# HpWang-whu/YOHO

Hardware: AMD Instinct MI355X
Metric: keypoints/sec (5000 kp x60 rot desc+YOHO-O) (higher is better)
Workload: dtype fp16x2 split (2^-22-accurate products, fp32 accumulate); 1 GPU

## Files before the change

yoho_amd/csrc/api.hip:

```cpp
#include "common.h"
#include <cstdarg>
#include <cstdio>
#include <cstring>
#include <cstdlib>
#include <cmath>
#include <vector>

namespace yoho {

static thread_local char g_err[512] = "";

void set_error(const char* fmt, ...) {
    va_list ap;
    va_start(ap, fmt);
    vsnprintf(g_err, sizeof(g_err), fmt, ap);
    va_end(ap);
}

void clear_error() { g_err[0] = 0; }

int hip_fail(hipError_t e, const char* what, const char* file, int line) {
    set_error("HIP error %d (%s) at %s:%d: %s", (int)e, hipGetErrorString(e), file, line, what);
    return YOHO_EHIP;
}
// ... 280 lines not shown
                const int g = outg[cfg * G + sl];
                slab[cfg * NTAP * G + tap * nslots + sl] = (g < 0 ? 0 : (int)N[g * NTAP + tap]) * 1024;
            }
    };
    std::vector<int> all(G); for (int i = 0; i < G; ++i) all[i] = i;
    std::vector<int> one(NTAP); for (int k = 0; k < NTAP; ++k) one[k] = N[k];
    std::vector<bool> in2(G, false);
    for (int k = 0; k < NTAP; ++k) for (int k2 = 0; k2 < NTAP; ++k2) in2[N[one[k] * NTAP + k2]] = true;
    std::vector<int> two; for (int g = 0; g < G; ++g) if (in2[g]) two.push_back(g);
    if (two.size() > 48) { set_error("2-hop cone of group element 0 has %zu > 48 elements", two.size()); delete c; return YOHO_EINVAL; }
    fill(CFG_FULL, all, 15, false);
    fill(CFG_C45, two, 12, false);
    fill(CFG_C13, one, 4, false);
    fill(CFG_C1, std::vector<int>{0}, 1, true);
    if ((rc = upload_slot_tables(slab.data(), outg.data(), c->tabs)) || (rc = gconv_init())) { delete c; return rc; }
    {
        std::vector<int> slab4(3 * 7 * 32, 0), unitg(3 * 32 * 2, -1);
        const std::vector<int>* lists[3] = {&all, &two, &one};
        for (int cfg = 0; cfg < 3; ++cfg) {
            const std::vector<int>& gl = *lists[cfg];
            int* ug = &unitg[cfg * 64];
            for (size_t k = 0; k < gl.size(); ++k) ug[k] = gl[k];
            for (int tp = 0; tp < 7; ++tp)
                for (int u = 0; u < 32; ++u)
                    for (int gs = 0; gs < 2; ++gs)
                        for (int h = 0; h < 2; ++h) {
                            int g = ug[2 * u + gs];
                            if (g < 0) g = ug[2 * u];
                            int tap = 2 * tp + h;
                            if (tap >= NTAP) tap = 2 * tp;
                            slab4[(cfg * 7 + tp) * 32 + u] |= (g < 0 ? 0 : (int)N[g * NTAP + tap]) << (8 * (2 * gs + h));
                        }
        }
        if ((rc = upload_slot_tables16(slab4.data(), unitg.data(), c->tabs)) || (rc = gconv16_init())) { delete c; return rc; }
    }
    c->gconv_mode = 4;
    c->partII_mode = 2;
    {
        auto is = [](const char* name, const char* val) { const char* e = std::getenv(name); return e && std::strcmp(e, val) == 0; };
        auto num = [](const char* name) { const char* e = std::getenv(name); return e ? std::atoi(e) : 0; };
        c->env.partII_tail_staged = is("YOHO_PARTII_TAIL", "staged");
        c->env.transfer_staged = is("YOHO_TRANSFER", "staged");
        c->env.xf_steal = !is("YOHO_XF_STEAL", "0");
        c->env.nn_splits = num("YOHO_NN_SPLITS");
        c->env.spconv_debug = num("YOHO_SPCONV_DEBUG");
        c->env.fcgf_f32 = is("YOHO_FCGF", "f32");
        c->env.fcgf_full_maps = is("YOHO_FCGF_MAPS", "full");
        c->env.fcgf_norm_staged = is("YOHO_FCGF_NORM", "staged");
        c->env.fcgf_heads_staged = is("YOHO_FCGF_HEADS", "staged");
        if (const char* e = std::getenv("YOHO_WS_LIMIT_MB")) c->env.ws_limit_mb = std::atoll(e);
        if (is("YOHO_PARTII_L1", "3")) c->env.partII_l1_variant = FG_TILE256_W8;
    }
    if (const char* m = std::getenv("YOHO_FCGF_CELLS")) c->fcgf_cell_sort = std::atoi(m);
    if (const char* m = std::getenv("YOHO_FCGF_SORT")) c->fcgf_parity_sort = std::strcmp(m, "0") == 0 ? 0 : 1;
    if (const char* m = std::getenv("YOHO_FCGF_COORDS")) c->fcgf_hash_coords = std::strcmp(m, "hash") == 0 ? 1 : 0;
    if (const char* m = std::getenv("YOHO_NN")) c->nn_prefilter = std::strcmp(m, "brute") == 0 ? 0 : 1;
    if (const char* m = std::getenv("YOHO_PARTII")) c->partII_mode = std::strcmp(m, "f32") == 0 ? 0 : (std::strcmp(m, "fp16x2") == 0 ? 2 : (std::strcmp(m, "cgemm") == 0 ? 3 : (std::strcmp(m, "cgemm8") == 0 ? 4 : 1)));
    if (const char* m = std::getenv("YOHO_PARTI_CHUNK")) {
        int ck = 0, ns = 1;
        if (std::sscanf(m, "%dx%d", &ck, &ns) >= 1 && ck >= 0 && (ns == 1 || ns == 2)) { c->partI_chunk = (ck + 255) / 256 * 256; c->partI_streams = ns; }
    }
    if (const char* m = std::getenv("YOHO_GCONV")) c->gconv_mode = std::strcmp(m, "f32") == 0 ? 0 : (std::strcmp(m, "bf16x3") == 0 ? 1 : (std::strcmp(m, "fp16x2") == 0 ? 3 : (std::strcmp(m, "fgemm") == 0 ? 4 : (std::strcmp(m, "fgemm256") == 0 ? 5 : (std::strcmp(m, "fgemm128") == 0 ? 6 : (std::strcmp(m, "fgemm8") == 0 ? 7 : 2))))));
    c->fb = new FourierBasis();
    if ((rc = build_fourier(N, P, *c->fb))) { delete c->fb; delete c; return rc; }
    {
        std::vector<float> fpad(2 * 64 * 64, 0.f);
        for (int s = 0; s < G; ++s)
// ... 839 lines not shown
```

yoho_amd/csrc/common.h:

```cpp
#pragma once
#include <hip/hip_runtime.h>
#include <stdint.h>
#include <stddef.h>
#include <initializer_list>
#include "yoho_hip.h"
#include "arena.h"

namespace yoho {

constexpr int G = 60;
constexpr int NTAP = 13;
constexpr int F = 32;
constexpr int TILE = 32;
constexpr int SLAB_FLOATS = 2 * TILE * 4;
constexpr int CHUNK_FLOATS = G * SLAB_FLOATS;

void set_error(const char* fmt, ...);
void clear_error();
inline bool yoho_misaligned(std::initializer_list<const void*> ps, unsigned mask) {
    for (const void* p : ps) if ((reinterpret_cast<uintptr_t>(p) & mask) != 0) return true;
    return false;
}
#define YOHO_NEED_ALIGNED(fn, mask, ...)                                                                                  \
    do {                                                                                                                  \
// ... 91 lines not shown
int gft_init();
int fgemm_init();
size_t fgemm_planes_bytes(int kppad, int cin);
void fgemm_qinfo(int* qi);
void fgemm_plane_offsets(int kppad, int cin, long long* off);
int pack_fgemm_weights(const FourierBasis& fb, const float* W, int cin, int cout, std::vector<unsigned short>& out, float* descale,
                       std::vector<unsigned short>* out8 = nullptr);
int pack_cgemm_weights(const float* W, int cin, int cout, int ntaps, std::vector<unsigned short>& out, float* descale, std::vector<unsigned short>& out8);
int cgemm_init();
int launch_cgemm(const Layer& L, const char* Bstages, int nslot, const unsigned char* slot, const unsigned char* outg, int nT32, int nTiles16,
                 char* out, hipStream_t s, int* rflag, const unsigned* amax);
int launch_gft16_invg(const float* in, float* res0, char* planesG, const int* slot_of, int nslot, const void* Ffrag, const float* bn_s,
                      const float* bn_t, int nTiles, int C8, int nCU, hipStream_t s, int* rflag, unsigned* amax);
int launch_fgemm(const Layer& L, const char* Bplanes, int kppad, int nT32, const float* res, float* out, int flags, hipStream_t s,
                 int* rflag = nullptr, FGemmBlocking blocking = FG_TILE128, const unsigned* amax = nullptr);
void build_gft16_frags(const FourierBasis& fb, std::vector<unsigned short>& out);
int gconv_layer(yoho_ctx* c, const float* x, int B, int cin, int cout, const float* W, const float* bias, int transpose, float* y,
                hipStream_t s);
int bn_stats(const float* x, int B, int C, float* mean, float* var, hipStream_t s);
int bn_relu_apply(const float* x, int B, int C, const float* scale, const float* shift, float* y, hipStream_t s);
int bn_relu_backward(const float* x, const float* y, const float* dy, int B, int C, const float* gamma, const float* mean, const float* rstd,
                     int batch_stats, float* dx, float* dgamma, float* dbeta, hipStream_t s);
int gconv_wgrad(yoho_ctx* c, const float* x, const float* dy, int B, int cin, int cout, float* dW, float* db, hipStream_t s);
struct FcgfNet;
int fcgf_load(FcgfNet** out, const yoho_fcgf_config* cfg, const float* const* t, int ntensors, bool f32_kernels);
void fcgf_free(FcgfNet* n);
int fcgf_forward(yoho_ctx* ctx, const FcgfNet* net, const int* coords0, int n0, const int* off_host, int nb, float* out, hipStream_t s);
int fcgf_voxelize(yoho_ctx* ctx, const double* pts, int n, const double* R_host, double voxel, int64_t* sel, int* coords, float* pts_sel,
                  int* count_host, hipStream_t s);
int fcgf_rotate_select(const double* pts, const double* R_host, const int64_t* sel, int m, float* out, hipStream_t s);
int fcgf_voxelize_batch(yoho_ctx* ctx, const double* pts, int n, const double* R_host, int nb, double voxel, int64_t* sel, int* coords,
                        float* pts_sel, int* counts_host, hipStream_t s);
int launch_cone1(const Layer& L, const char* X, int nTiles32, int nTiles16, const float* res, float* out, const int* n0, hipStream_t s, float* part = nullptr);
int gft16_init();
int launch_gft16(const float* in, float* out32, char* planes, int kppad, const void* Ffrag, const float* bn_s, const float* bn_t, int nTiles,
                 int C8, int nCU, hipStream_t s, int B = 0, int* rflag = nullptr, int variant = 2, int* ctr = nullptr, unsigned* amax = nullptr);
int launch_gft16_invp(const float* in, float* res0, char* planes16, int nTiles16, const void* Ffrag, const float* bn_s, const float* bn_t,
                      int nTiles, int C8, int nCU, hipStream_t s, int* rflag = nullptr);
int launch_head2(const float* s0, const float* s1, const float* s2, const float* s3, const int64_t* pre_idx, const int* P, const float* bn_s,
                 const float* bn_t, int M, int nTiles, char* planes, int kppad, const void* Ffrag, hipStream_t s,
                 const int64_t* const* ridx = nullptr, int istride = 1, int* rflag = nullptr);
int launch_head16(const float* x, int B, int nTiles, char* planes, int kppad, const void* Ffrag, hipStream_t s, const float* x1 = nullptr,
                  int B0 = 0, int* rflag = nullptr);
int launch_gconvf(const Layer& L, const float* X, int nTiles, const float* res, float* out, int flags, hipStream_t s);
int launch_gft(int mode, const float* in, float* out, const float* Fpad, const float* bn_s, const float* bn_t, int nTiles, int C8, hipStream_t s);
int upload_slot_tables16(const int* slab4_h, const int* unitg_h, SlotTables& t);
int gconv16_init();
int launch_gconv16(const Layer& L, const char* X, int nTiles, const float* res, float* out_raw, char* out_act, int flags, hipStream_t s,
                   int cfg = 0, float* out_raw32 = nullptr, float* out_act32 = nullptr, int npl = 3, int* rflag = nullptr);
int launch_pack16_partII(const float* s0, const float* s1, const float* s2, const float* s3, const int64_t* pre_idx, const int* P,
                         const float* bn_s, const float* bn_t, int M, int nTiles16, char* out, hipStream_t s, int npl = 3, int* rflag = nullptr);
int launch_pack16_partI(const float* x, int B, int nTiles, char* out, hipStream_t s, int npl = 3, int* rflag = nullptr);
int launch_group_mean_np(const float* eqv, int B, float* out, hipStream_t s);
int launch_pack_partII(const float* s0, const float* s1, const float* s2, const float* s3, const int64_t* pre_idx,
                       const int* P, const float* bn_s, const float* bn_t, int M, int nTiles, float* out, hipStream_t s);
int launch_quat_norm(const float* y, int M, float* quat, hipStream_t s);

struct MfArgs {
    const float* a; const float* b;
    int Na, Nb;
    float* na2; float* nb2;
    _Float16* a16; _Float16* b16;
    unsigned* rowmin; unsigned* colmin;
    unsigned long long* keysA; unsigned long long* keysB;
    unsigned* maxn2;
    int* bad;
// ... 159 lines not shown
```

yoho_amd/csrc/cone1.hip:

```cpp
#include <hip/hip_runtime.h>
#include <type_traits>

#include "common.h"

namespace yoho {

typedef float floatx16 __attribute__((ext_vector_type(16)));
typedef float floatx4 __attribute__((ext_vector_type(4)));
typedef unsigned uintx4 __attribute__((ext_vector_type(4)));
typedef _Float16 halfx8 __attribute__((ext_vector_type(8)));
typedef const __attribute__((address_space(1))) void* gptr_t;
typedef __attribute__((address_space(3))) void* lptr_t;

constexpr int C1_CHUNK = 30720;
constexpr int C1_PLANE = 15360;
constexpr int C1_STAGE = 2 * 2 * 14 * 256;
constexpr int C1_UNITS = C1_STAGE / 1024;

struct Cone1Args {
    const char* X;
    const char* Wp;
    const float* bias;
    const float* res;
    float* out;
    int nTiles32, nTiles16, cin8, cout8;
    float* part;
    float descale;
    int n0[14];
};

__device__ __forceinline__ floatx16 mfma_c1(uintx4 a, uintx4 b, floatx16 c) {
    union { uintx4 u; halfx8 h; } ca, cb;
    ca.u = a; cb.u = b;
    return __builtin_amdgcn_mfma_f32_32x32x16_f16(ca.h, cb.h, c, 0, 0, 0);
}

template <int I, int N, typename Fn>
__device__ __forceinline__ void sfor_c1(Fn&& fn) {
    if constexpr (I < N) { fn(std::integral_constant<int, I>{}); sfor_c1<I + 1, N>(fn); }
}

__global__ __launch_bounds__(256, 1) void cone1_kernel(Cone1Args a) {
    __shared__ __attribute__((aligned(16))) char smem[3 * C1_STAGE];
    __shared__ int n0s[16];
    const int tid = threadIdx.x, lane = tid & 63;
    const int w = __builtin_amdgcn_readfirstlane(tid >> 6);
    const int nog = a.cout8 / 16;
    const int cn = a.cin8 / (int)gridDim.y, c0 = (int)blockIdx.y * cn;
    const int tile32 = blockIdx.x / nog, og = blockIdx.x - tile32 * nog;
    const int ob = og * 4 + w;
    if (tid < 14) n0s[tid] = a.n0[tid];
    __syncthreads();

    long long soff[4];
#pragma unroll
    for (int i = 0; i < 4; ++i) {
        const int u = w + 4 * i < C1_UNITS ? w + 4 * i : w + 4 * (i - 1);
        const int slot = u * 4 + (lane >> 4);
        const int pl = slot / 28, r = slot - pl * 28, ht = r / 14, k = r - ht * 14;
        int t16 = 2 * tile32 + ht;
        t16 = t16 < a.nTiles16 ? t16 : a.nTiles16 - 1;
        soff[i] = (long long)t16 * a.cin8 * C1_CHUNK + pl * C1_PLANE + n0s[k] * 256 + (lane & 15) * 16;
    }
    auto stage = [&](int c8, char* dst) {
#pragma unroll
        for (int i = 0; i < 4; ++i) {
            const int u = w + 4 * i < C1_UNITS ? w + 4 * i : w + 4 * (i - 1);
            __builtin_amdgcn_global_load_lds((gptr_t)(a.X + soff[i] + (long long)(c0 + c8) * C1_CHUNK), (lptr_t)(dst + u * 1024), 16, 0, 0);
        }
    };

    floatx16 acc[3];
#pragma unroll
    for (int j = 0; j < 3; ++j)
#pragma unroll
        for (int r = 0; r < 16; ++r) acc[j][r] = 0.f;

    const int lane_b = ((lane >> 4) & 1) * (14 * 256) + (lane >> 5) * 256 + (lane & 15) * 16;
    const uintx4* Wl = reinterpret_cast<const uintx4*>(a.Wp) + (size_t)ob * a.cin8 * (7 * 2 * 64) + lane;

    constexpr int RING = 3;
    uintx4 wreg[RING][7][2];
    auto loadW = [&](int c8, uintx4 (&wr)[7][2]) {
        const uintx4* Wn = Wl + (size_t)(c0 + c8) * (7 * 2 * 64);
#pragma unroll
        for (int tp = 0; tp < 7; ++tp) { wr[tp][0] = Wn[(tp * 2) * 64]; wr[tp][1] = Wn[(tp * 2 + 1) * 64]; }
    };
    auto compute = [&](const char* cur, const uintx4 (&wr)[7][2]) {
        const unsigned base = (unsigned)(size_t)(cur + lane_b);
        uintx4 bh[7], bl[7];
#pragma unroll
        for (int tp = 0; tp < 7; ++tp)
            asm volatile("ds_read_b128 %0, %2 offset:%3\n\tds_read_b128 %1, %2 offset:%4"
                         : "=&v"(bh[tp]), "=&v"(bl[tp]) : "v"(base), "n"(tp * 512), "n"(tp * 512 + 2 * 14 * 256) : "memory");
        asm volatile("s_waitcnt lgkmcnt(0)"
                     : "+v"(bh[0]), "+v"(bh[1]), "+v"(bh[2]), "+v"(bh[3]), "+v"(bh[4]), "+v"(bh[5]), "+v"(bh[6]),
                       "+v"(bl[0]), "+v"(bl[1]), "+v"(bl[2]), "+v"(bl[3]), "+v"(bl[4]), "+v"(bl[5]), "+v"(bl[6]) :: "memory");
#pragma unroll
        for (int tp = 0; tp < 7; ++tp) {
            acc[0] = mfma_c1(wr[tp][1], bh[tp], acc[0]);
            acc[1] = mfma_c1(wr[tp][0], bl[tp], acc[1]);
            acc[2] = mfma_c1(wr[tp][0], bh[tp], acc[2]);
        }
    };
    auto top = [&]() {
        __builtin_amdgcn_s_waitcnt(0x4F72);
        asm volatile("s_waitcnt lgkmcnt(0)" ::: "memory");
        __builtin_amdgcn_s_barrier();
        __builtin_amdgcn_sched_barrier(0);
    };
    auto stage_of = [&](int c8) { return smem + (c8 % RING) * C1_STAGE; };
    const int last = cn - 1;
    auto clamp = [&](int c8) { return c8 <= last ? c8 : last; };
    loadW(clamp(0), wreg[0]); stage(clamp(0), stage_of(0));
    loadW(clamp(1), wreg[1]); stage(clamp(1), stage_of(1));
    const int nmain = (cn / RING) * RING;
    for (int c8 = 0; c8 < nmain; c8 += RING) {
        sfor_c1<0, RING>([&](auto jc) {
            constexpr int jj = decltype(jc)::value;
            const int c = c8 + jj;
            top();
            loadW(clamp(c + RING - 1), wreg[(jj + RING - 1) % RING]);
            stage(clamp(c + RING - 1), stage_of(c + RING - 1));
            compute(stage_of(c), wreg[jj]);
        });
    }
    sfor_c1<0, RING - 1>([&](auto jc) {
        constexpr int jj = decltype(jc)::value;
        if (nmain + jj <= last) {
            top();
            loadW(last, wreg[(jj + RING - 1) % RING]);
            stage(last, stage_of(nmain + jj + RING - 1));
            compute(stage_of(nmain + jj), wreg[jj]);
        }
    });
    asm volatile("s_waitcnt vmcnt(0)" ::: "memory");

    const int kp32 = lane & 31, half = lane >> 5;
#pragma unroll
    for (int q = 0; q < 4; ++q) {
        const int ch = ob * 32 + q * 8 + half * 4;
        floatx4 val;
        val.x = (acc[0][4 * q + 0] + acc[1][4 * q + 0]) + acc[2][4 * q + 0];
        val.y = (acc[0][4 * q + 1] + acc[1][4 * q + 1]) + acc[2][4 * q + 1];
        val.z = (acc[0][4 * q + 2] + acc[1][4 * q + 2]) + acc[2][4 * q + 2];
        val.w = (acc[0][4 * q + 3] + acc[1][4 * q + 3]) + acc[2][4 * q + 3];
        if (gridDim.y > 1) {
            *reinterpret_cast<floatx4*>(a.part + ((((size_t)blockIdx.y * a.nTiles32 + tile32) * a.cout8 + ob * 4 + q) * 64 + lane) * 4) = val;
            continue;
        }
        val *= a.descale;
        val += *reinterpret_cast<const floatx4*>(a.bias + ch);
        const size_t off = (((((size_t)tile32 * a.cout8 + ob * 4 + q) * G + 0) * 2 + half) * TILE + kp32) * 4;
        if (a.res) val += *reinterpret_cast<const floatx4*>(a.res + off);
        *reinterpret_cast<floatx4*>(a.out + off) = val;
    }
}

int launch_cone1(const Layer& L, const char* X, int nTiles32, int nTiles16, const float* res, float* out, const int* n0, hipStream_t s, float* part) {
    if (L.cout_pad % 128 || !L.wph || L.cin % 32) { set_error("cone1: needs cout %% 128 == 0, cin %% 32 == 0 and fp16x2 weights"); return YOHO_EINVAL; }
    Cone1Args a;
    a.X = X; a.Wp = reinterpret_cast<const char*>(L.wph); a.bias = L.bias; a.res = res; a.out = out; a.part = part;
    if (part && (L.cin / 8) % 2) { set_error("cone1: K split needs an even number of channel chunks"); return YOHO_EINVAL; }
    a.nTiles32 = nTiles32; a.nTiles16 = nTiles16; a.cin8 = L.cin / 8; a.cout8 = L.cout_pad / 8; a.descale = L.wph_descale;
    for (int k = 0; k < 13; ++k) a.n0[k] = n0[k];
    a.n0[13] = n0[0];
    if (nTiles32 == 0) return 0;
    hipLaunchKernelGGL(cone1_kernel, dim3(nTiles32 * (a.cout8 / 16), part ? 2 : 1), dim3(256), 0, s, a);
    HIPCHK(hipGetLastError());
    return 0;
}

}
```

yoho_amd/csrc/gconv.hip:

```cpp
#include "common.h"

namespace yoho {

typedef float floatx16 __attribute__((ext_vector_type(16)));
typedef float floatx4 __attribute__((ext_vector_type(4)));

constexpr int CHUNK_BYTES = CHUNK_FLOATS * 4;
constexpr int LDS_BYTES = 2 * CHUNK_BYTES;

typedef const __attribute__((address_space(4))) int* cint_p;

int upload_slot_tables(const int* slab_h, const int* outg_h, SlotTables& t) {
    HIPCHK(hipMalloc((void**)&t.slabtab, sizeof(int) * NCFG * NTAP * G));
    HIPCHK(hipMalloc((void**)&t.outg, sizeof(int) * NCFG * G));
    HIPCHK(hipMemcpy(t.slabtab, slab_h, sizeof(int) * NCFG * NTAP * G, hipMemcpyHostToDevice));
    HIPCHK(hipMemcpy(t.outg, outg_h, sizeof(int) * NCFG * G, hipMemcpyHostToDevice));
    return 0;
}

typedef const __attribute__((address_space(1))) void* gptr_t;
typedef __attribute__((address_space(3))) void* lptr_t;

__device__ __forceinline__ void stage_chunk(const float* src, char* dst, int w, int lane, int npieces) {
    for (int p = w; p < npieces; p += 4) {
// ... 88 lines not shown
template <int GPW, bool OSPLIT>
static int launch_t(const ConvArgs& a, int flags, int nstage, int cfg, hipStream_t s) {
    const int grid = a.nTiles * a.nOB;
    hipLaunchKernelGGL((gconv_kernel<GPW, OSPLIT>), dim3(grid), dim3(256), LDS_BYTES, s, a, flags, nstage, cfg);
    HIPCHK(hipGetLastError());
    return 0;
}

template <int GPW, bool OSPLIT>
static int init_t() {
    HIPCHK(hipFuncSetAttribute(reinterpret_cast<const void*>(&gconv_kernel<GPW, OSPLIT>),
                               hipFuncAttributeMaxDynamicSharedMemorySize, LDS_BYTES));
    return 0;
}

struct MlpArgs {
    const float* X;
    const float *WA, *biasA, *sA, *tA;
    const float *WB, *biasB, *sB, *tB;
    const float *WC, *biasC;
    int cinA8, obA, obB, M;
    float* quat;
    const float* part; const float* biasP; const float* resP; float descaleP; int nTiles;
};

__device__ __forceinline__ floatx4 quat_unit(floatx4 q) {
#pragma clang fp contract(off)
    const float n = sqrtf(((q.x * q.x + q.y * q.y) + q.z * q.z) + q.w * q.w);
    floatx4 o;
    o.x = q.x / n; o.y = q.y / n; o.z = q.z / n; o.w = q.w / n;
    return o;
}

__global__ __launch_bounds__(256, 1) void mlp_head_kernel(MlpArgs a) {
    extern __shared__ __attribute__((aligned(16))) char smem[];
    const int tid = threadIdx.x, lane = tid & 63;
    const int w = __builtin_amdgcn_readfirstlane(tid >> 6);
    const int tile = blockIdx.x;
    char* sX = smem;
    char* sA = sX + a.cinA8 * 1024;
    char* sB = sA + a.obA * 4 * 1024;
    const int half = lane >> 5;
    if (a.part) {
        for (int p = w; p < a.cinA8; p += 4) {
            const size_t o0 = (((size_t)tile * a.cinA8 + p) * 64 + lane) * 4, o1 = o0 + (size_t)a.nTiles * a.cinA8 * 256;
            floatx4 val = *reinterpret_cast<const floatx4*>(a.part + o0) + *reinterpret_cast<const floatx4*>(a.part + o1);
            val *= a.descaleP;
            val += *reinterpret_cast<const floatx4*>(a.biasP + p * 8 + half * 4);
            if (a.resP) val += *reinterpret_cast<const floatx4*>(a.resP + ((size_t)tile * a.cinA8 + p) * CHUNK_FLOATS + lane * 4);
            *reinterpret_cast<floatx4*>(sX + p * 1024 + lane * 16) = val;
        }
    } else {
        const float* Xt = a.X + (size_t)tile * a.cinA8 * CHUNK_FLOATS;
        for (int p = w; p < a.cinA8; p += 4)
            __builtin_amdgcn_global_load_lds((gptr_t)(Xt + (size_t)p * CHUNK_FLOATS + lane * 4), (lptr_t)(sX + p * 1024), 16, 0, 0);
    }
    {
        floatx16 acc[4];
#pragma unroll
        for (int j = 0; j < 4; ++j)
#pragma unroll
            for (int i = 0; i < 16; ++i) acc[j][i] = 0.f;
        const floatx4* W0 = reinterpret_cast<const floatx4*>(a.WA) + (size_t)w * a.cinA8 * 64 + lane;
        const size_t wstride = (size_t)4 * a.cinA8 * 64;
        floatx4 wn[4];
#pragma unroll
        for (int j = 0; j < 4; ++j) wn[j] = W0[j * wstride];
        asm volatile("s_waitcnt vmcnt(0)" ::: "memory");
        __syncthreads();
        for (int c8 = 0; c8 < a.cinA8; ++c8) {
            floatx4 wc[4];
#pragma unroll
            for (int j = 0; j < 4; ++j) wc[j] = wn[j];
            if (c8 + 1 < a.cinA8) {
#pragma unroll
                for (int j = 0; j < 4; ++j) wn[j] = W0[j * wstride + (size_t)(c8 + 1) * 64];
            }
            const floatx4 xf = *reinterpret_cast<const floatx4*>(sX + c8 * 1024 + lane * 16);
#pragma unroll
            for (int j = 0; j < 4; ++j) {
                acc[j] = __builtin_amdgcn_mfma_f32_32x32x2f32(wc[j].x, xf.x, acc[j], 0, 0, 0);
                acc[j] = __builtin_amdgcn_mfma_f32_32x32x2f32(wc[j].y, xf.y, acc[j], 0, 0, 0);
                acc[j] = __builtin_amdgcn_mfma_f32_32x32x2f32(wc[j].z, xf.z, acc[j], 0, 0, 0);
                acc[j] = __builtin_amdgcn_mfma_f32_32x32x2f32(wc[j].w, xf.w, acc[j], 0, 0, 0);
            }
        }
#pragma unroll
        for (int j = 0; j < 4; ++j) {
            const int ob = w + 4 * j;
#pragma unroll
            for (int q = 0; q < 4; ++q) {
                const int ch = ob * 32 + q * 8 + half * 4;
                floatx4 val;
                val.x = acc[j][4 * q + 0]; val.y = acc[j][4 * q + 1];
                val.z = acc[j][4 * q + 2]; val.w = acc[j][4 * q + 3];
                val += *reinterpret_cast<const floatx4*>(a.biasA + ch);
                const floatx4 sc = *reinterpret_cast<const floatx4*>(a.sA + ch);
                const floatx4 sh = *reinterpret_cast<const floatx4*>(a.tA + ch);
                floatx4 y = val * sc + sh;
                y.x = fmaxf(y.x, 0.f); y.y = fmaxf(y.y, 0.f); y.z = fmaxf(y.z, 0.f); y.w = fmaxf(y.w, 0.f);
                *reinterpret_cast<floatx4*>(sA + (ob * 4 + q) * 1024 + lane * 16) = y;
            }
        }
    }
    __syncthreads();
    {
        floatx16 acc;
#pragma unroll
        for (int i = 0; i < 16; ++i) acc[i] = 0.f;
        const int cin8 = a.obA * 4;
        const floatx4* W0 = reinterpret_cast<const floatx4*>(a.WB) + (size_t)w * cin8 * 64 + lane;
        floatx4 wr[4];
#pragma unroll
        for (int d = 0; d < 4; ++d) wr[d] = W0[(size_t)(d < cin8 ? d : cin8 - 1) * 64];
        for (int c0 = 0; c0 < cin8; c0 += 4) {
#pragma unroll
            for (int d = 0; d < 4; ++d) {
                const int c8 = c0 + d;
                const floatx4 wc = wr[d];
                const int nx = c8 + 4 < cin8 ? c8 + 4 : cin8 - 1;
                wr[d] = W0[(size_t)nx * 64];
                const floatx4 xf = *reinterpret_cast<const floatx4*>(sA + c8 * 1024 + lane * 16);
                acc = __builtin_amdgcn_mfma_f32_32x32x2f32(wc.x, xf.x, acc, 0, 0, 0);
                acc = __builtin_amdgcn_mfma_f32_32x32x2f32(wc.y, xf.y, acc, 0, 0, 0);
                acc = __builtin_amdgcn_mfma_f32_32x32x2f32(wc.z, xf.z, acc, 0, 0, 0);
                acc = __builtin_amdgcn_mfma_f32_32x32x2f32(wc.w, xf.w, acc, 0, 0, 0);
            }
        }
#pragma unroll
        for (int q = 0; q < 4; ++q) {
            const int ch = w * 32 + q * 8 + half * 4;
            floatx4 val;
            val.x = acc[4 * q + 0]; val.y = acc[4 * q + 1];
            val.z = acc[4 * q + 2]; val.w = acc[4 * q + 3];
            val += *reinterpret_cast<const floatx4*>(a.biasB + ch);
            const floatx4 sc = *reinterpret_cast<const floatx4*>(a.sB + ch);
            const floatx4 sh = *reinterpret_cast<const floatx4*>(a.tB + ch);
            floatx4 y = val * sc + sh;
            y.x = fmaxf(y.x, 0.f); y.y = fmaxf(y.y, 0.f); y.z = fmaxf(y.z, 0.f); y.w = fmaxf(y.w, 0.f);
            *reinterpret_cast<floatx4*>(sB + (w * 4 + q) * 1024 + lane * 16) = y;
        }
    }
    __syncthreads();
    if (w == 0) {
        floatx16 acc;
#pragma unroll
        for (int i = 0; i < 16; ++i) acc[i] = 0.f;
        const int cin8 = a.obB * 4;
        const floatx4* W0 = reinterpret_cast<const floatx4*>(a.WC) + lane;
        floatx4 wr[4];
#pragma unroll
        for (int d = 0; d < 4; ++d) wr[d] = W0[(size_t)(d < cin8 ? d : cin8 - 1) * 64];
        for (int c0 = 0; c0 < cin8; c0 += 4) {
#pragma unroll
            for (int d = 0; d < 4; ++d) {
                const int c8 = c0 + d;
                const floatx4 wc = wr[d];
                const int nx = c8 + 4 < cin8 ? c8 + 4 : cin8 - 1;
                wr[d] = W0[(size_t)nx * 64];
                const floatx4 xf = *reinterpret_cast<const floatx4*>(sB + c8 * 1024 + lane * 16);
                acc = __builtin_amdgcn_mfma_f32_32x32x2f32(wc.x, xf.x, acc, 0, 0, 0);
                acc = __builtin_amdgcn_mfma_f32_32x32x2f32(wc.y, xf.y, acc, 0, 0, 0);
                acc = __builtin_amdgcn_mfma_f32_32x32x2f32(wc.z, xf.z, acc, 0, 0, 0);
                acc = __builtin_amdgcn_mfma_f32_32x32x2f32(wc.w, xf.w, acc, 0, 0, 0);
            }
        }
        floatx4 val;
        val.x = acc[0]; val.y = acc[1]; val.z = acc[2]; val.w = acc[3];
        val += *reinterpret_cast<const floatx4*>(a.biasC + half * 4);
        const int m = tile * TILE + (lane & 31);
        if (half == 0 && m < a.M) *reinterpret_cast<floatx4*>(a.quat + (size_t)m * 4) = quat_unit(val);
    }
}

bool mlp_head_supported(const Layer& A, const Layer& B, const Layer& C) {
    return A.ntaps == 1 && B.ntaps == 1 && C.ntaps == 1 && A.cin == 256 && A.cout_pad == 512 && B.cin == 512 && B.cout_pad == 128 &&
           C.cin == 128 && C.cout_pad == 32;
}

int launch_mlp_head(const Layer& A, const Layer& B, const Layer& C, const float* X, int nTiles, int M, float* quat, hipStream_t s,
                    const float* part, const Layer* P, const float* res) {
    MlpArgs a;
    a.X = X;
    a.part = part; a.biasP = P ? P->bias : nullptr; a.resP = res; a.descaleP = P ? P->wph_descale : 1.f; a.nTiles = nTiles;
    if (part && !P) { set_error("mlp head: partial sums without their layer"); return YOHO_EINVAL; }
    a.WA = A.wp; a.biasA = A.bias; a.sA = A.bn_s; a.tA = A.bn_t;
    a.WB = B.wp; a.biasB = B.bias; a.sB = B.bn_s; a.tB = B.bn_t;
    a.WC = C.wp; a.biasC = C.bias;
    a.cinA8 = A.cin / 8; a.obA = A.cout_pad / 32; a.obB = B.cout_pad / 32; a.M = M;
    a.quat = quat;
    const int lds = (a.cinA8 + a.obA * 4 + a.obB * 4) * 1024;
    hipLaunchKernelGGL(mlp_head_kernel, dim3(nTiles), dim3(256), lds, s, a);
    HIPCHK(hipGetLastError());
    return 0;
}

int gconv_init() {
    int rc;
    HIPCHK(hipFuncSetAttribute(reinterpret_cast<const void*>(&mlp_head_kernel), hipFuncAttributeMaxDynamicSharedMemorySize, 112 * 1024));
    if ((rc = init_t<15, false>())) return rc;
    if ((rc = init_t<12, false>())) return rc;
    if ((rc = init_t<4, false>())) return rc;
    if ((rc = init_t<1, false>())) return rc;
    if ((rc = init_t<1, true>())) return rc;
    return 0;
}

int launch_gconv(const ConvArgs& a, int gpw, int flags, hipStream_t s) {
    if (!a.slabtab || !a.outg) { set_error("launch_gconv: the layer carries no slot tables"); return YOHO_EINVAL; }
    int nstage = G;
    switch (gpw) {
        case 15: return launch_t<15, false>(a, flags, nstage, CFG_FULL, s);
        case 12: return launch_t<12, false>(a, flags, nstage, CFG_C45, s);
        case 4:  return launch_t<4, false>(a, flags, nstage, CFG_C13, s);
        case 1:  return launch_t<1, false>(a, flags, a.ntaps == 1 ? 1 : nstage, CFG_C1, s);
        case -1: return launch_t<1, true>(a, flags, a.ntaps == 1 ? 1 : nstage, CFG_C1, s);
        default: set_error("launch_gconv: unsupported slots-per-wave %d", gpw); return YOHO_EINVAL;
    }
}

}
```

Baseline: 1.893 million keypoints/s.

## Process two tiles per cone1 block and software-pipeline the MLP head weights

The cone1 kernel now handles two 32-keypoint tiles per block, so each wave reuses its register-resident weights across both tiles. The LDS stage doubles, becoming dynamic shared memory set up in a new init call, and the counted DMA waits are retuned to match. Separately, the MLP head kernel is specialised to fixed 256-512-128 shapes with deeper weight register rings, prefetched bias/BN parameters, LDS read-ahead, and scheduling barriers. Costs are higher register and LDS pressure, half as many cone1 blocks for the GPU to spread across CUs, and an error for other MLP shapes.

```diff
diff --git a/yoho_amd/csrc/api.hip b/yoho_amd/csrc/api.hip
--- a/yoho_amd/csrc/api.hip
+++ b/yoho_amd/csrc/api.hip
@@ -336,7 +336,7 @@
                             slab4[(cfg * 7 + tp) * 32 + u] |= (g < 0 ? 0 : (int)N[g * NTAP + tap]) << (8 * (2 * gs + h));
                         }
         }
-        if ((rc = upload_slot_tables16(slab4.data(), unitg.data(), c->tabs)) || (rc = gconv16_init())) { delete c; return rc; }
+        if ((rc = upload_slot_tables16(slab4.data(), unitg.data(), c->tabs)) || (rc = gconv16_init()) || (rc = cone1_init())) { delete c; return rc; }
     }
     c->gconv_mode = 4;
     c->partII_mode = 2;
diff --git a/yoho_amd/csrc/common.h b/yoho_amd/csrc/common.h
--- a/yoho_amd/csrc/common.h
+++ b/yoho_amd/csrc/common.h
@@ -147,6 +147,7 @@
 int fcgf_voxelize_batch(yoho_ctx* ctx, const double* pts, int n, const double* R_host, int nb, double voxel, int64_t* sel, int* coords,
                         float* pts_sel, int* counts_host, hipStream_t s);
 int launch_cone1(const Layer& L, const char* X, int nTiles32, int nTiles16, const float* res, float* out, const int* n0, hipStream_t s, float* part = nullptr);
+int cone1_init();
 int gft16_init();
 int launch_gft16(const float* in, float* out32, char* planes, int kppad, const void* Ffrag, const float* bn_s, const float* bn_t, int nTiles,
                  int C8, int nCU, hipStream_t s, int B = 0, int* rflag = nullptr, int variant = 2, int* ctr = nullptr, unsigned* amax = nullptr);
diff --git a/yoho_amd/csrc/cone1.hip b/yoho_amd/csrc/cone1.hip
--- a/yoho_amd/csrc/cone1.hip
+++ b/yoho_amd/csrc/cone1.hip
@@ -14,8 +14,13 @@
 
 constexpr int C1_CHUNK = 30720;
 constexpr int C1_PLANE = 15360;
-constexpr int C1_STAGE = 2 * 2 * 14 * 256;
+constexpr int C1_BLOCK = 2 * 2 * 14 * 256;
+constexpr int C1_STAGE = 2 * C1_BLOCK;
 constexpr int C1_UNITS = C1_STAGE / 1024;
+constexpr int C1_PIECES = C1_UNITS / 4;
+constexpr int C1_RING = 3;
+constexpr int C1_LDS = C1_RING * C1_STAGE + 64;
+static_assert(C1_UNITS % 4 == 0, "every wave issues the same number of DMA pieces: the counted wait depends on it");
 
 struct Cone1Args {
     const char* X;
@@ -41,45 +46,44 @@
 }
 
 __global__ __launch_bounds__(256, 1) void cone1_kernel(Cone1Args a) {
-    __shared__ __attribute__((aligned(16))) char smem[3 * C1_STAGE];
-    __shared__ int n0s[16];
+    extern __shared__ __attribute__((aligned(16))) char smem[];
+    int* n0s = reinterpret_cast<int*>(smem + C1_RING * C1_STAGE);
     const int tid = threadIdx.x, lane = tid & 63;
     const int w = __builtin_amdgcn_readfirstlane(tid >> 6);
     const int nog = a.cout8 / 16;
     const int cn = a.cin8 / (int)gridDim.y, c0 = (int)blockIdx.y * cn;
-    const int tile32 = blockIdx.x / nog, og = blockIdx.x - tile32 * nog;
+    const int tile64 = blockIdx.x / nog, og = blockIdx.x - tile64 * nog;
     const int ob = og * 4 + w;
     if (tid < 14) n0s[tid] = a.n0[tid];
     __syncthreads();
 
-    long long soff[4];
-#pragma unroll
-    for (int i = 0; i < 4; ++i) {
-        const int u = w + 4 * i < C1_UNITS ? w + 4 * i : w + 4 * (i - 1);
-        const int slot = u * 4 + (lane >> 4);
-        const int pl = slot / 28, r = slot - pl * 28, ht = r / 14, k = r - ht * 14;
-        int t16 = 2 * tile32 + ht;
+    long long soff[C1_PIECES];
+#pragma unroll
+    for (int i = 0; i < C1_PIECES; ++i) {
+        const int slot = (w + 4 * i) * 4 + (lane >> 4);
+        const int cb = slot / 56, r = slot - cb * 56, pl = r / 28, r2 = r - pl * 28, ht = r2 / 14, k = r2 - ht * 14;
+        int t16 = 2 * (2 * tile64 + cb) + ht;
         t16 = t16 < a.nTiles16 ? t16 : a.nTiles16 - 1;
         soff[i] = (long long)t16 * a.cin8 * C1_CHUNK + pl * C1_PLANE + n0s[k] * 256 + (lane & 15) * 16;
     }
     auto stage = [&](int c8, char* dst) {
 #pragma unroll
-        for (int i = 0; i < 4; ++i) {
-            const int u = w + 4 * i < C1_UNITS ? w + 4 * i : w + 4 * (i - 1);
-            __builtin_amdgcn_global_load_lds((gptr_t)(a.X + soff[i] + (long long)(c0 + c8) * C1_CHUNK), (lptr_t)(dst + u * 1024), 16, 0, 0);
-        }
-    };
-
-    floatx16 acc[3];
-#pragma unroll
-    for (int j = 0; j < 3; ++j)
-#pragma unroll
-        for (int r = 0; r < 16; ++r) acc[j][r] = 0.f;
+        for (int i = 0; i < C1_PIECES; ++i)
+            __builtin_amdgcn_global_load_lds((gptr_t)(a.X + soff[i] + (long long)(c0 + c8) * C1_CHUNK), (lptr_t)(dst + (w + 4 * i) * 1024), 16, 0, 0);
+    };
+
+    floatx16 acc[2][3];
+#pragma unroll
+    for (int cb = 0; cb < 2; ++cb)
+#pragma unroll
+        for (int j = 0; j < 3; ++j)
+#pragma unroll
+            for (int r = 0; r < 16; ++r) acc[cb][j][r] = 0.f;
 
     const int lane_b = ((lane >> 4) & 1) * (14 * 256) + (lane >> 5) * 256 + (lane & 15) * 16;
     const uintx4* Wl = reinterpret_cast<const uintx4*>(a.Wp) + (size_t)ob * a.cin8 * (7 * 2 * 64) + lane;
 
-    constexpr int RING = 3;
+    constexpr int RING = C1_RING;
     uintx4 wreg[RING][7][2];
     auto loadW = [&](int c8, uintx4 (&wr)[7][2]) {
         const uintx4* Wn = Wl + (size_t)(c0 + c8) * (7 * 2 * 64);
@@ -88,23 +92,36 @@
     };
     auto compute = [&](const char* cur, const uintx4 (&wr)[7][2]) {
         const unsigned base = (unsigned)(size_t)(cur + lane_b);
-        uintx4 bh[7], bl[7];
-#pragma unroll
-        for (int tp = 0; tp < 7; ++tp)
-            asm volatile("ds_read_b128 %0, %2 offset:%3\n\tds_read_b128 %1, %2 offset:%4"
-                         : "=&v"(bh[tp]), "=&v"(bl[tp]) : "v"(base), "n"(tp * 512), "n"(tp * 512 + 2 * 14 * 256) : "memory");
+        uintx4 bh[2][7], bl[2][7];
+#pragma unroll
+        for (int cb = 0; cb < 2; ++cb)
+#pragma unroll
+            for (int tp = 0; tp < 7; ++tp)
+                asm volatile("ds_read_b128 %0, %2 offset:%3\n\tds_read_b128 %1, %2 offset:%4"
+                             : "=&v"(bh[cb][tp]), "=&v"(bl[cb][tp])
+                             : "v"(base), "n"(cb * C1_BLOCK + tp * 512), "n"(cb * C1_BLOCK + tp * 512 + 2 * 14 * 256) : "memory");
+        asm volatile("s_waitcnt lgkmcnt(14)"
+                     : "+v"(bh[0][0]), "+v"(bh[0][1]), "+v"(bh[0][2]), "+v"(bh[0][3]), "+v"(bh[0][4]), "+v"(bh[0][5]), "+v"(bh[0][6]),
+                       "+v"(bl[0][0]), "+v"(bl[0][1]), "+v"(bl[0][2]), "+v"(bl[0][3]), "+v"(bl[0][4]), "+v"(bl[0][5]), "+v"(bl[0][6]) :: "memory");
+#pragma unroll
+        for (int tp = 0; tp < 7; ++tp) {
+            acc[0][0] = mfma_c1(wr[tp][1], bh[0][tp], acc[0][0]);
+            acc[0][1] = mfma_c1(wr[tp][0], bl[0][tp], acc[0][1]);
+            acc[0][2] = mfma_c1(wr[tp][0], bh[0][tp], acc[0][2]);
+        }
         asm volatile("s_waitcnt lgkmcnt(0)"
-                     : "+v"(bh[0]), "+v"(bh[1]), "+v"(bh[2]), "+v"(bh[3]), "+v"(bh[4]), "+v"(bh[5]), "+v"(bh[6]),
-                       "+v"(bl[0]), "+v"(bl[1]), "+v"(bl[2]), "+v"(bl[3]), "+v"(bl[4]), "+v"(bl[5]), "+v"(bl[6]) :: "memory");
+                     : "+v"(bh[1][0]), "+v"(bh[1][1]), "+v"(bh[1][2]), "+v"(bh[1][3]), "+v"(bh[1][4]), "+v"(bh[1][5]), "+v"(bh[1][6]),
+                       "+v"(bl[1][0]), "+v"(bl[1][1]), "+v"(bl[1][2]), "+v"(bl[1][3]), "+v"(bl[1][4]), "+v"(bl[1][5]), "+v"(bl[1][6]) :: "memory");
 #pragma unroll
         for (int tp = 0; tp < 7; ++tp) {
-            acc[0] = mfma_c1(wr[tp][1], bh[tp], acc[0]);
-            acc[1] = mfma_c1(wr[tp][0], bl[tp], acc[1]);
-            acc[2] = mfma_c1(wr[tp][0], bh[tp], acc[2]);
-        }
-    };
+            acc[1][0] = mfma_c1(wr[tp][1], bh[1][tp], acc[1][0]);
+            acc[1][1] = mfma_c1(wr[tp][0], bl[1][tp], acc[1][1]);
+            acc[1][2] = mfma_c1(wr[tp][0], bh[1][tp], acc[1][2]);
+        }
+    };
+    static_assert(14 + C1_PIECES == 21, "the wait below is vmcnt(21)");
     auto top = [&]() {
-        __builtin_amdgcn_s_waitcnt(0x4F72);
+        __builtin_amdgcn_s_waitcnt(0x4F75);
         asm volatile("s_waitcnt lgkmcnt(0)" ::: "memory");
         __builtin_amdgcn_s_barrier();
         __builtin_amdgcn_sched_barrier(0);
@@ -113,6 +130,7 @@
     const int last = cn - 1;
     auto clamp = [&](int c8) { return c8 <= last ? c8 : last; };
     loadW(clamp(0), wreg[0]); stage(clamp(0), stage_of(0));
+    __builtin_amdgcn_sched_barrier(0);
     loadW(clamp(1), wreg[1]); stage(clamp(1), stage_of(1));
     const int nmain = (cn / RING) * RING;
     for (int c8 = 0; c8 < nmain; c8 += RING) {
@@ -138,23 +156,33 @@
 
     const int kp32 = lane & 31, half = lane >> 5;
 #pragma unroll
-    for (int q = 0; q < 4; ++q) {
-        const int ch = ob * 32 + q * 8 + half * 4;
-        floatx4 val;
-        val.x = (acc[0][4 * q + 0] + acc[1][4 * q + 0]) + acc[2][4 * q + 0];
-        val.y = (acc[0][4 * q + 1] + acc[1][4 * q + 1]) + acc[2][4 * q + 1];
-        val.z = (acc[0][4 * q + 2] + acc[1][4 * q + 2]) + acc[2][4 * q + 2];
-        val.w = (acc[0][4 * q + 3] + acc[1][4 * q + 3]) + acc[2][4 * q + 3];
-        if (gridDim.y > 1) {
-            *reinterpret_cast<floatx4*>(a.part + ((((size_t)blockIdx.y * a.nTiles32 + tile32) * a.cout8 + ob * 4 + q) * 64 + lane) * 4) = val;
-            continue;
-        }
-        val *= a.descale;
-        val += *reinterpret_cast<const floatx4*>(a.bias + ch);
-        const size_t off = (((((size_t)tile32 * a.cout8 + ob * 4 + q) * G + 0) * 2 + half) * TILE + kp32) * 4;
-        if (a.res) val += *reinterpret_cast<const floatx4*>(a.res + off);
-        *reinterpret_cast<floatx4*>(a.out + off) = val;
+    for (int cb = 0; cb < 2; ++cb) {
+        const int tile32 = 2 * tile64 + cb;
+        if (tile32 >= a.nTiles32) continue;
+#pragma unroll
+        for (int q = 0; q < 4; ++q) {
+            const int ch = ob * 32 + q * 8 + half * 4;
+            floatx4 val;
+            val.x = (acc[cb][0][4 * q + 0] + acc[cb][1][4 * q + 0]) + acc[cb][2][4 * q + 0];
+            val.y = (acc[cb][0][4 * q + 1] + acc[cb][1][4 * q + 1]) + acc[cb][2][4 * q + 1];
+            val.z = (acc[cb][0][4 * q + 2] + acc[cb][1][4 * q + 2]) + acc[cb][2][4 * q + 2];
+            val.w = (acc[cb][0][4 * q + 3] + acc[cb][1][4 * q + 3]) + acc[cb][2][4 * q + 3];
+            if (gridDim.y > 1) {
+                *reinterpret_cast<floatx4*>(a.part + ((((size_t)blockIdx.y * a.nTiles32 + tile32) * a.cout8 + ob * 4 + q) * 64 + lane) * 4) = val;
+                continue;
+            }
+            val *= a.descale;
+            val += *reinterpret_cast<const floatx4*>(a.bias + ch);
+            const size_t off = (((((size_t)tile32 * a.cout8 + ob * 4 + q) * G + 0) * 2 + half) * TILE + kp32) * 4;
+            if (a.res) val += *reinterpret_cast<const floatx4*>(a.res + off);
+            *reinterpret_cast<floatx4*>(a.out + off) = val;
+        }
     }
+}
+
+int cone1_init() {
+    HIPCHK(hipFuncSetAttribute(reinterpret_cast<const void*>(&cone1_kernel), hipFuncAttributeMaxDynamicSharedMemorySize, C1_LDS));
+    return 0;
 }
 
 int launch_cone1(const Layer& L, const char* X, int nTiles32, int nTiles16, const float* res, float* out, const int* n0, hipStream_t s, float* part) {
@@ -166,7 +194,7 @@
     for (int k = 0; k < 13; ++k) a.n0[k] = n0[k];
     a.n0[13] = n0[0];
     if (nTiles32 == 0) return 0;
-    hipLaunchKernelGGL(cone1_kernel, dim3(nTiles32 * (a.cout8 / 16), part ? 2 : 1), dim3(256), 0, s, a);
+    hipLaunchKernelGGL(cone1_kernel, dim3((nTiles32 + 1) / 2 * (a.cout8 / 16), part ? 2 : 1), dim3(256), C1_LDS, s, a);
     HIPCHK(hipGetLastError());
     return 0;
 }
diff --git a/yoho_amd/csrc/gconv.hip b/yoho_amd/csrc/gconv.hip
--- a/yoho_amd/csrc/gconv.hip
+++ b/yoho_amd/csrc/gconv.hip
@@ -144,71 +144,127 @@
     return o;
 }
 
+constexpr int MLP_CA8 = 32, MLP_OBA = 16, MLP_OBB = 4;
+constexpr int MLP_RA = 4;
+constexpr int MLP_RB = 8;
+static_assert(MLP_CA8 % (4 * MLP_RA) == 0 && (MLP_OBA * 4) % MLP_RB == 0 && (MLP_OBB * 4) % MLP_RB == 0, "whole rings");
+
 __global__ __launch_bounds__(256, 1) void mlp_head_kernel(MlpArgs a) {
     extern __shared__ __attribute__((aligned(16))) char smem[];
     const int tid = threadIdx.x, lane = tid & 63;
     const int w = __builtin_amdgcn_readfirstlane(tid >> 6);
     const int tile = blockIdx.x;
     char* sX = smem;
-    char* sA = sX + a.cinA8 * 1024;
-    char* sB = sA + a.obA * 4 * 1024;
+    char* sA = sX + MLP_CA8 * 1024;
+    char* sB = sA + MLP_OBA * 4 * 1024;
     const int half = lane >> 5;
+    constexpr int cinB8 = MLP_OBA * 4, cinC8 = MLP_OBB * 4;
+    const floatx4* WA0 = reinterpret_cast<const floatx4*>(a.WA) + (size_t)w * MLP_CA8 * 64 + lane;
+    const floatx4* WB0 = reinterpret_cast<const floatx4*>(a.WB) + (size_t)w * cinB8 * 64 + lane;
+    const floatx4* WC0 = reinterpret_cast<const floatx4*>(a.WC) + lane;
+    constexpr size_t wstride = (size_t)4 * MLP_CA8 * 64;
+    floatx4 wrA[MLP_RA][4], wrB[MLP_RB], wrC[MLP_RB];
+#pragma unroll
+    for (int d = 0; d < MLP_RA; ++d)
+#pragma unroll
+        for (int j = 0; j < 4; ++j) wrA[d][j] = WA0[j * wstride + (size_t)d * 64];
     if (a.part) {
-        for (int p = w; p < a.cinA8; p += 4) {
-            const size_t o0 = (((size_t)tile * a.cinA8 + p) * 64 + lane) * 4, o1 = o0 + (size_t)a.nTiles * a.cinA8 * 256;
-            floatx4 val = *reinterpret_cast<const floatx4*>(a.part + o0) + *reinterpret_cast<const floatx4*>(a.part + o1);
+        constexpr int NP = MLP_CA8 / 4;
+        floatx4 p0[NP], p1[NP], rs[NP], bs[NP];
+#pragma unroll
+        for (int i = 0; i < NP; ++i) {
+            const int p = w + 4 * i;
+            const size_t o0 = (((size_t)tile * MLP_CA8 + p) * 64 + lane) * 4, o1 = o0 + (size_t)a.nTiles * MLP_CA8 * 256;
+            p0[i] = *reinterpret_cast<const floatx4*>(a.part + o0);
+            p1[i] = *reinterpret_cast<const floatx4*>(a.part + o1);
+            bs[i] = *reinterpret_cast<const floatx4*>(a.biasP + p * 8 + half * 4);
+        }
+        if (a.resP) {
+#pragma unroll
+            for (int i = 0; i < NP; ++i)
+                rs[i] = *reinterpret_cast<const floatx4*>(a.resP + ((size_t)tile * MLP_CA8 + w + 4 * i) * CHUNK_FLOATS + lane * 4);
+        }
+#pragma unroll
+        for (int d = 0; d < MLP_RB; ++d) { wrB[d] = WB0[(size_t)d * 64]; wrC[d] = WC0[(size_t)d * 64]; }
+#pragma unroll
+        for (int i = 0; i < NP; ++i) {
+            floatx4 val = p0[i] + p1[i];
             val *= a.descaleP;
-            val += *reinterpret_cast<const floatx4*>(a.biasP + p * 8 + half * 4);
-            if (a.resP) val += *reinterpret_cast<const floatx4*>(a.resP + ((size_t)tile * a.cinA8 + p) * CHUNK_FLOATS + lane * 4);
-            *reinterpret_cast<floatx4*>(sX + p * 1024 + lane * 16) = val;
+            val += bs[i];
+            if (a.resP) val += rs[i];
+            *reinterpret_cast<floatx4*>(sX + (w + 4 * i) * 1024 + lane * 16) = val;
         }
     } else {
-        const float* Xt = a.X + (size_t)tile * a.cinA8 * CHUNK_FLOATS;
-        for (int p = w; p < a.cinA8; p += 4)
+        const float* Xt = a.X + (size_t)tile * MLP_CA8 * CHUNK_FLOATS;
+        for (int p = w; p < MLP_CA8; p += 4)
             __builtin_amdgcn_global_load_lds((gptr_t)(Xt + (size_t)p * CHUNK_FLOATS + lane * 4), (lptr_t)(sX + p * 1024), 16, 0, 0);
-    }
+#pragma unroll
+        for (int d = 0; d < MLP_RB; ++d) { wrB[d] = WB0[(size_t)d * 64]; wrC[d] = WC0[(size_t)d * 64]; }
+    }
+    asm volatile("s_waitcnt vmcnt(0)" ::: "memory");
+    __syncthreads();
+    floatx4 pbB[4], psB[4], ptB[4], pbC;
     {
         floatx16 acc[4];
 #pragma unroll
         for (int j = 0; j < 4; ++j)
 #pragma unroll
             for (int i = 0; i < 16; ++i) acc[j][i] = 0.f;
-        const floatx4* W0 = reinterpret_cast<const floatx4*>(a.WA) + (size_t)w * a.cinA8 * 64 + lane;
-        const size_t wstride = (size_t)4 * a.cinA8 * 64;
-        floatx4 wn[4];
-#pragma unroll
-        for (int j = 0; j < 4; ++j) wn[j] = W0[j * wstride];
-        asm volatile("s_waitcnt vmcnt(0)" ::: "memory");
-        __syncthreads();
-        for (int c8 = 0; c8 < a.cinA8; ++c8) {
-            floatx4 wc[4];
-#pragma unroll
-            for (int j = 0; j < 4; ++j) wc[j] = wn[j];
-            if (c8 + 1 < a.cinA8) {
-#pragma unroll
-                for (int j = 0; j < 4; ++j) wn[j] = W0[j * wstride + (size_t)(c8 + 1) * 64];
-            }
-            const floatx4 xf = *reinterpret_cast<const floatx4*>(sX + c8 * 1024 + lane * 16);
-#pragma unroll
-            for (int j = 0; j < 4; ++j) {
-                acc[j] = __builtin_amdgcn_mfma_f32_32x32x2f32(wc[j].x, xf.x, acc[j], 0, 0, 0);
-                acc[j] = __builtin_amdgcn_mfma_f32_32x32x2f32(wc[j].y, xf.y, acc[j], 0, 0, 0);
-                acc[j] = __builtin_amdgcn_mfma_f32_32x32x2f32(wc[j].z, xf.z, acc[j], 0, 0, 0);
-                acc[j] = __builtin_amdgcn_mfma_f32_32x32x2f32(wc[j].w, xf.w, acc[j], 0, 0, 0);
-            }
-        }
+        floatx4 xn = *reinterpret_cast<const floatx4*>(sX + lane * 16);
+#pragma unroll
+        for (int c0 = 0; c0 < MLP_CA8; c0 += MLP_RA) {
+#pragma unroll
+            for (int d = 0; d < MLP_RA; ++d) {
+                const int c8 = c0 + d;
+                floatx4 wc[4];
+#pragma unroll
+                for (int j = 0; j < 4; ++j) wc[j] = wrA[d][j];
+                const int nx = c8 + MLP_RA < MLP_CA8 ? c8 + MLP_RA : MLP_CA8 - 1;
+#pragma unroll
+                for (int j = 0; j < 4; ++j) wrA[d][j] = WA0[j * wstride + (size_t)nx * 64];
+                const floatx4 xf = xn;
+                xn = *reinterpret_cast<const floatx4*>(sX + (c8 + 1 < MLP_CA8 ? c8 + 1 : c8) * 1024 + lane * 16);
+                __builtin_amdgcn_sched_barrier(0);
+#pragma unroll
+                for (int j = 0; j < 4; ++j) {
+                    acc[j] = __builtin_amdgcn_mfma_f32_32x32x2f32(wc[j].x, xf.x, acc[j], 0, 0, 0);
+                    acc[j] = __builtin_amdgcn_mfma_f32_32x32x2f32(wc[j].y, xf.y, acc[j], 0, 0, 0);
+                    acc[j] = __builtin_amdgcn_mfma_f32_32x32x2f32(wc[j].z, xf.z, acc[j], 0, 0, 0);
+                    acc[j] = __builtin_amdgcn_mfma_f32_32x32x2f32(wc[j].w, xf.w, acc[j], 0, 0, 0);
+                }
+                __builtin_amdgcn_sched_barrier(0);
+            }
+        }
+        floatx4 pb[4][4], ps[4][4], pt[4][4];
+#pragma unroll
+        for (int j = 0; j < 4; ++j)
+#pragma unroll
+            for (int q = 0; q < 4; ++q) {
+                const int ch = (w + 4 * j) * 32 + q * 8 + half * 4;
+                pb[j][q] = *reinterpret_cast<const floatx4*>(a.biasA + ch);
+                ps[j][q] = *reinterpret_cast<const floatx4*>(a.sA + ch);
+                pt[j][q] = *reinterpret_cast<const floatx4*>(a.tA + ch);
+            }
+#pragma unroll
+        for (int q = 0; q < 4; ++q) {
+            const int ch = w * 32 + q * 8 + half * 4;
+            pbB[q] = *reinterpret_cast<const floatx4*>(a.biasB + ch);
+            psB[q] = *reinterpret_cast<const floatx4*>(a.sB + ch);
+            ptB[q] = *reinterpret_cast<const floatx4*>(a.tB + ch);
+        }
+        pbC = *reinterpret_cast<const floatx4*>(a.biasC + half * 4);
+        __builtin_amdgcn_sched_barrier(0);
 #pragma unroll
         for (int j = 0; j < 4; ++j) {
             const int ob = w + 4 * j;
 #pragma unroll
             for (int q = 0; q < 4; ++q) {
-                const int ch = ob * 32 + q * 8 + half * 4;
                 floatx4 val;
                 val.x = acc[j][4 * q + 0]; val.y = acc[j][4 * q + 1];
                 val.z = acc[j][4 * q + 2]; val.w = acc[j][4 * q + 3];
-                val += *reinterpret_cast<const floatx4*>(a.biasA + ch);
-                const floatx4 sc = *reinterpret_cast<const floatx4*>(a.sA + ch);
-                const floatx4 sh = *reinterpret_cast<const floatx4*>(a.tA + ch);
+                val += pb[j][q];
+                const floatx4 sc = ps[j][q];
+                const floatx4 sh = pt[j][q];
                 floatx4 y = val * sc + sh;
                 y.x = fmaxf(y.x, 0.f); y.y = fmaxf(y.y, 0.f); y.z = fmaxf(y.z, 0.f); y.w = fmaxf(y.w, 0.f);
                 *reinterpret_cast<floatx4*>(sA + (ob * 4 + q) * 1024 + lane * 16) = y;
@@ -220,34 +276,33 @@
         floatx16 acc;
 #pragma unroll
         for (int i = 0; i < 16; ++i) acc[i] = 0.f;
-        const int cin8 = a.obA * 4;
-        const floatx4* W0 = reinterpret_cast<const floatx4*>(a.WB) + (size_t)w * cin8 * 64 + lane;
-        floatx4 wr[4];
-#pragma unroll
-        for (int d = 0; d < 4; ++d) wr[d] = W0[(size_t)(d < cin8 ? d : cin8 - 1) * 64];
-        for (int c0 = 0; c0 < cin8; c0 += 4) {
-#pragma unroll
-            for (int d = 0; d < 4; ++d) {
+        floatx4 xn = *reinterpret_cast<const floatx4*>(sA + lane * 16);
+#pragma unroll
+        for (int c0 = 0; c0 < cinB8; c0 += MLP_RB) {
+#pragma unroll
+            for (int d = 0; d < MLP_RB; ++d) {
                 const int c8 = c0 + d;
-                const floatx4 wc = wr[d];
-                const int nx = c8 + 4 < cin8 ? c8 + 4 : cin8 - 1;
-                wr[d] = W0[(size_t)nx * 64];
-                const floatx4 xf = *reinterpret_cast<const floatx4*>(sA + c8 * 1024 + lane * 16);
+                const floatx4 wc = wrB[d];
+                const int nx = c8 + MLP_RB < cinB8 ? c8 + MLP_RB : cinB8 - 1;
+                wrB[d] = WB0[(size_t)nx * 64];
+                const floatx4 xf = xn;
+                xn = *reinterpret_cast<const floatx4*>(sA + (c8 + 1 < cinB8 ? c8 + 1 : c8) * 1024 + lane * 16);
+                __builtin_amdgcn_sched_barrier(0);
                 acc = __builtin_amdgcn_mfma_f32_32x32x2f32(wc.x, xf.x, acc, 0, 0, 0);
                 acc = __builtin_amdgcn_mfma_f32_32x32x2f32(wc.y, xf.y, acc, 0, 0, 0);
                 acc = __builtin_amdgcn_mfma_f32_32x32x2f32(wc.z, xf.z, acc, 0, 0, 0);
                 acc = __builtin_amdgcn_mfma_f32_32x32x2f32(wc.w, xf.w, acc, 0, 0, 0);
+                __builtin_amdgcn_sched_barrier(0);
             }
         }
 #pragma unroll
         for (int q = 0; q < 4; ++q) {
-            const int ch = w * 32 + q * 8 + half * 4;
             floatx4 val;
             val.x = acc[4 * q + 0]; val.y = acc[4 * q + 1];
             val.z = acc[4 * q + 2]; val.w = acc[4 * q + 3];
-            val += *reinterpret_cast<const floatx4*>(a.biasB + ch);
-            const floatx4 sc = *reinterpret_cast<const floatx4*>(a.sB + ch);
-            const floatx4 sh = *reinterpret_cast<const floatx4*>(a.tB + ch);
+            val += pbB[q];
+            const floatx4 sc = psB[q];
+            const floatx4 sh = ptB[q];
             floatx4 y = val * sc + sh;
             y.x = fmaxf(y.x, 0.f); y.y = fmaxf(y.y, 0.f); y.z = fmaxf(y.z, 0.f); y.w = fmaxf(y.w, 0.f);
             *reinterpret_cast<floatx4*>(sB + (w * 4 + q) * 1024 + lane * 16) = y;
@@ -258,28 +313,28 @@
         floatx16 acc;
 #pragma unroll
         for (int i = 0; i < 16; ++i) acc[i] = 0.f;
-        const int cin8 = a.obB * 4;
-        const floatx4* W0 = reinterpret_cast<const floatx4*>(a.WC) + lane;
-        floatx4 wr[4];
-#pragma unroll
-        for (int d = 0; d < 4; ++d) wr[d] = W0[(size_t)(d < cin8 ? d : cin8 - 1) * 64];
-        for (int c0 = 0; c0 < cin8; c0 += 4) {
-#pragma unroll
-            for (int d = 0; d < 4; ++d) {
+        floatx4 xn = *reinterpret_cast<const floatx4*>(sB + lane * 16);
+#pragma unroll
+        for (int c0 = 0; c0 < cinC8; c0 += MLP_RB) {
+#pragma unroll
+            for (int d = 0; d < MLP_RB; ++d) {
                 const int c8 = c0 + d;
-                const floatx4 wc = wr[d];
-                const int nx = c8 + 4 < cin8 ? c8 + 4 : cin8 - 1;
-                wr[d] = W0[(size_t)nx * 64];
-                const floatx4 xf = *reinterpret_cast<const floatx4*>(sB + c8 * 1024 + lane * 16);
+                const floatx4 wc = wrC[d];
+                const int nx = c8 + MLP_RB < cinC8 ? c8 + MLP_RB : cinC8 - 1;
+                wrC[d] = WC0[(size_t)nx * 64];
+                const floatx4 xf = xn;
+                xn = *reinterpret_cast<const floatx4*>(sB + (c8 + 1 < cinC8 ? c8 + 1 : c8) * 1024 + lane * 16);
+                __builtin_amdgcn_sched_barrier(0);
                 acc = __builtin_amdgcn_mfma_f32_32x32x2f32(wc.x, xf.x, acc, 0, 0, 0);
                 acc = __builtin_amdgcn_mfma_f32_32x32x2f32(wc.y, xf.y, acc, 0, 0, 0);
                 acc = __builtin_amdgcn_mfma_f32_32x32x2f32(wc.z, xf.z, acc, 0, 0, 0);
                 acc = __builtin_amdgcn_mfma_f32_32x32x2f32(wc.w, xf.w, acc, 0, 0, 0);
+                __builtin_amdgcn_sched_barrier(0);
             }
         }
         floatx4 val;
         val.x = acc[0]; val.y = acc[1]; val.z = acc[2]; val.w = acc[3];
-        val += *reinterpret_cast<const floatx4*>(a.biasC + half * 4);
+        val += pbC;
         const int m = tile * TILE + (lane & 31);
         if (half == 0 && m < a.M) *reinterpret_cast<floatx4*>(a.quat + (size_t)m * 4) = quat_unit(val);
     }
@@ -301,6 +356,7 @@
     a.WC = C.wp; a.biasC = C.bias;
     a.cinA8 = A.cin / 8; a.obA = A.cout_pad / 32; a.obB = B.cout_pad / 32; a.M = M;
     a.quat = quat;
+    if (a.cinA8 != MLP_CA8 || a.obA != MLP_OBA || a.obB != MLP_OBB) { set_error("mlp head: shapes other than 256-512-128-4"); return YOHO_EINVAL; }
     const int lds = (a.cinA8 + a.obA * 4 + a.obB * 4) * 1024;
     hipLaunchKernelGGL(mlp_head_kernel, dim3(nTiles), dim3(256), lds, s, a);
     HIPCHK(hipGetLastError());
```

Result: no change. 1.899 million keypoints/s, median of 6 (+0.3%).
